# kkty/kmer-sets-compression

Measured on AMD Instinct MI355X. Metric: Mk-mers/s processed in kmerset-multiple-compress; bytes/k-mer after SPSS, higher is better.
Workload: dtype u32

## Files before the change

kmer-sets-compression_amd/csrc/ksh_encode.hip:

```cpp
#include "ksh_internal.h"
#include "ksh_dsu.h"
#include "ksh_kmer.h"

#include <algorithm>
#include <cstddef>
#include <cstdlib>
#include <string>

namespace ksh {

#ifndef KSH_RULER_SHIFT
#define KSH_RULER_SHIFT 5
#endif
constexpr int kRulerShift = KSH_RULER_SHIFT;
constexpr uint32_t kRulerEvery = 1u << kRulerShift;

constexpr uint32_t kNone = 0xFFFFFFFFu;
constexpr uint32_t kMulti = 0xFFFFFFFEu;

#ifndef KSH_JUMP_HOPS
#define KSH_JUMP_HOPS 4
#endif
constexpr int kJumpHops = KSH_JUMP_HOPS;

#ifdef KSH_TRACE
__device__ unsigned long long* g_probe_trace = nullptr;
__device__ long long g_probe_trace_rows = 0;
#define KSH_PMARK(which, m)                                                                              \
  do {                                                                                                   \
    if (g_probe_trace && threadIdx.x == 0 && int64_t(blockIdx.x) < g_probe_trace_rows)                    \
      g_probe_trace[((which) * g_probe_trace_rows + blockIdx.x) * 16 + (m)] = __builtin_amdgcn_s_memtime(); \
  } while (0)
#define KSH_PMARK_WAVE(which)                                                                            \
  do {                                                                                                   \
    if (g_probe_trace && threadIdx.x % 64 == 0 && threadIdx.x / 64 < 16 && int64_t(blockIdx.x) < g_probe_trace_rows) \
      g_probe_trace[((which) * g_probe_trace_rows + blockIdx.x) * 16 + threadIdx.x / 64] = __builtin_amdgcn_s_memtime(); \
  } while (0)
#else
#define KSH_PMARK(which, m) do { } while (0)
#define KSH_PMARK_WAVE(which) do { } while (0)
#endif

template <typename KeyT>
__global__ __launch_bounds__(256) void k_fine_index(const int64_t* __restrict__ off,
                                                     const KeyT* __restrict__ keys, int key_bits,
                                                     int fine_bits, uint32_t* __restrict__ fine,
                                                     int64_t n_buckets) {
  extern __shared__ uint32_t s_fine[];
  const int64_t b = blockIdx.x;
  const int64_t lo = off[b], hi = off[b + 1];
  const int kSlices = 1 << fine_bits;
  const int sh = key_bits - fine_bits;
  uint32_t* f = fine + (b << fine_bits);
  if (lo == hi) {
    for (int sub = threadIdx.x; sub < kSlices; sub += 256) f[sub] = uint32_t(lo);
  } else {
    constexpr int kAhead = 4;
    for (int64_t base = lo; base < hi; base += 256 * kAhead) {
      KeyT cur_key[kAhead], prev_key[kAhead];
#pragma unroll
      for (int u = 0; u < kAhead; u++) {
        const int64_t i = base + u * 256 + threadIdx.x;
        if (i < hi) {
          cur_key[u] = keys[i];
          prev_key[u] = i > lo ? keys[i - 1] : KeyT(0);
        }
      }
#pragma unroll
      for (int u = 0; u < kAhead; u++) {
        const int64_t i = base + u * 256 + threadIdx.x;
        if (i < hi) {
          const int cur = int(uint64_t(cur_key[u]) >> sh);
          const int prev = i > lo ? int(uint64_t(prev_key[u]) >> sh) : -1;
          for (int sub = prev + 1; sub <= cur; sub++) s_fine[sub] = uint32_t(i);
        }
      }
    }
    const int last = int(uint64_t(keys[hi - 1]) >> sh);
    for (int sub = last + 1 + int(threadIdx.x); sub < kSlices; sub += 256) s_fine[sub] = uint32_t(hi);
    __syncthreads();
    for (int sub = threadIdx.x; sub < kSlices; sub += 256) f[sub] = s_fine[sub];
  }
  if (b == n_buckets - 1 && threadIdx.x == 0) fine[n_buckets << fine_bits] = uint32_t(hi);
}

template <typename KeyT>
__global__ __launch_bounds__(256) void k_coarse_index(DevSet<KeyT> set, int64_t n_entries, uint32_t* __restrict__ coarse) {
  const int64_t e = int64_t(blockIdx.x) * blockDim.x + threadIdx.x;
  if (e >= n_entries) return;
  const int64_t t = e << kCoarseShift;
  coarse[e] = uint32_t(set.bucket_search(t < set.n ? t : set.n - 1));
}

template <typename KeyT, bool kDirected, typename F>
__device__ __forceinline__ void for_side_neighbours(const DevSet<KeyT>& set, uint64_t x, uint64_t rx,
                                                    int64_t t, int side, F f) {
  const int k = set.k;
  if (kDirected) {
    if (side) {
      set.for_group4(kmer_next(x, k, 0), [&](int64_t idx) {
        if (idx != t) f(idx, 0u);
      });
    } else {
#pragma unroll
      for (int c = 0; c < 4; c++) {
        const uint64_t z = kmer_prev(x, k, c);
        if (z == x) continue;
        const int64_t idx = set.find(z);
        if (idx >= 0) f(idx, 0u);
      }
    }
    return;
  }
  set.for_group4(kmer_next(side ? x : rx, k, 0), [&](int64_t idx) {
    if (idx != t) f(idx, side ? 0u : 1u);
  });
  const uint64_t base = side ? rx : x;
#pragma unroll
  for (int c = 0; c < 4; c++) {
    const uint64_t z = kmer_prev(base, k, c);
    if (revcomp(z, k) < z) continue;
    if (z == x) continue;
    const int64_t idx = set.find(z);
    if (idx >= 0) f(idx, side ? 1u : 0u);
  }
}

template <typename KeyT, bool kDirected>
__global__ __launch_bounds__(256) void k_adjacency(DevSet<KeyT> set, uint32_t* __restrict__ nbr,
                                                    int* __restrict__ self_rc) {
  __shared__ int64_t s_bucket[2];
  const int64_t t = int64_t(blockIdx.x) * blockDim.x + threadIdx.x;
  const uint64_t x = set.kmer_in_block(t, s_bucket);
  if (t >= set.n) return;
  const uint64_t rx = kDirected ? 0 : revcomp(x, set.k);
  if (!kDirected && rx == x) *self_rc = 1;
  int cnt[2] = {0, 0};
  uint32_t single[2] = {kNone, kNone};
#pragma unroll
  for (int side = 0; side < 2; side++)
    for_side_neighbours<KeyT, kDirected>(set, x, rx, t, side, [&](int64_t idx, uint32_t same) {
      cnt[side]++;
      single[side] = (uint32_t(idx) << 1) | same;
    });
  nbr[2 * t] = cnt[0] == 0 ? kNone : (cnt[0] == 1 ? single[0] : kMulti);
  nbr[2 * t + 1] = cnt[1] == 0 ? kNone : (cnt[1] == 1 ? single[1] : kMulti);
}

template <typename KeyT, bool kDirected>
__global__ __launch_bounds__(256) void k_link_cut(DevSet<KeyT> set, uint32_t* __restrict__ nbr) {
  const int64_t t = int64_t(blockIdx.x) * blockDim.x + threadIdx.x;
  if (t >= set.n) return;
  const uint2 mine = reinterpret_cast<const uint2*>(nbr)[t];
  if (mine.x != kMulti && mine.y != kMulti) return;
  const uint64_t x = set.kmer(t);
  const uint64_t rx = kDirected ? 0 : revcomp(x, set.k);
  for (int side = 0; side < 2; side++) {
    if ((side ? mine.y : mine.x) != kMulti) continue;
    for_side_neighbours<KeyT, kDirected>(set, x, rx, t, side, [&](int64_t idx, uint32_t same) {
      uint32_t* facing = nbr + 2 * idx + (same ? side : side ^ 1);
      if (*reinterpret_cast<volatile uint32_t*>(facing) < kMulti) *reinterpret_cast<volatile uint32_t*>(facing) = kNone;
    });
    nbr[2 * t + side] = kNone;
  }
}

template <typename KeyT>
struct __attribute__((aligned(8))) RcRecord {
  KeyT key;
  uint32_t t;
};

template <typename KeyT>
__global__ __launch_bounds__(1024) void k_rc_hist(const KeyT* __restrict__ keys, int64_t n, int k, int key_bits,
                                                   int nbits, int64_t per_row,
                                                   uint32_t* __restrict__ hist_matrix) {
  extern __shared__ uint32_t lds_hist[];
  const int nb = 1 << nbits;
  for (int b = threadIdx.x; b < nb; b += blockDim.x) lds_hist[b] = 0u;
  __syncthreads();
  const int64_t t_begin = int64_t(blockIdx.x) * per_row;
  const int64_t t_end = min(t_begin + per_row, n);
  const int low_bits = 2 * k - 2 - nbits;
  for (int64_t t = t_begin + threadIdx.x; t < t_end; t += blockDim.x) {
    const uint64_t rx = revcomp(uint64_t(keys[t]), k);
    atomicAdd(&lds_hist[uint32_t(rx >> low_bits) & uint32_t(nb - 1)], 1u);
  }
  __syncthreads();
  uint32_t* my_row = hist_matrix + int64_t(blockIdx.x) * nb;
  for (int b = threadIdx.x; b < nb; b += blockDim.x) my_row[b] = lds_hist[b];
}

constexpr int kColTeams = 16;
__global__ __launch_bounds__(64 * kColTeams) void k_rc_columns(uint32_t* __restrict__ hist_matrix, int64_t n_rows,
                                                                int nb, int64_t* __restrict__ totals) {
  __shared__ uint32_t team_total[kColTeams][64];
  const int lane = threadIdx.x & 63, team = threadIdx.x >> 6;
  const int b = blockIdx.x * 64 + lane;
  const int64_t per_team = (n_rows + kColTeams - 1) / kColTeams;
  const int64_t g0 = min(int64_t(team) * per_team, n_rows), g1 = min(g0 + per_team, n_rows);
  uint32_t run = 0;
  if (b < nb)
    for (int64_t g = g0; g < g1; g++) run += hist_matrix[g * nb + b];
  team_total[team][lane] = run;
  __syncthreads();
  if (b >= nb) return;
  uint32_t before = 0, all = 0;
#pragma unroll
  for (int t2 = 0; t2 < kColTeams; t2++) {
    const uint32_t v = team_total[t2][lane];
    if (t2 < team) before += v;
    all += v;
  }
  run = before;
  for (int64_t g = g0; g < g1; g++) {
    uint32_t* cell = hist_matrix + g * nb + b;
    const uint32_t c = *cell;
    *cell = run;
    run += c;
  }
  if (team == 0) totals[b] = all;
}

template <typename KeyT>
__global__ __launch_bounds__(1024) void k_rc_scatter(DevSet<KeyT> set, int nbits, int round_bits, int round,
                                                      int64_t per_row,
                                                      const uint32_t* __restrict__ hist_matrix,
                                                      const int64_t* __restrict__ goff,
                                                      RcRecord<KeyT>* __restrict__ rec) {
  extern __shared__ uint32_t lds_hist[];
  const int nb = 1 << nbits;
  const uint32_t* my_row = hist_matrix + int64_t(blockIdx.x) * nb;
  for (int b = threadIdx.x; b < nb; b += blockDim.x) lds_hist[b] = uint32_t(goff[b]) + my_row[b];
  const int64_t t_begin = int64_t(blockIdx.x) * per_row;
  const int64_t t_end = min(t_begin + per_row, set.n);
  __syncthreads();
  if (t_begin >= t_end) return;
  const int64_t b_first = set.bucket_of(t_begin), b_last = set.bucket_of(t_end - 1);
  const int k = set.k, low_bits = 2 * set.k - 2 - nbits;
  const uint64_t low_mask = (uint64_t(1) << low_bits) - 1;
  for (int64_t t = t_begin + threadIdx.x; t < t_end; t += blockDim.x) {
    const uint64_t key = uint64_t(set.keys[t]);
    const uint32_t grp = uint32_t(revcomp(key, k) >> low_bits) & uint32_t(nb - 1);
    if (int(grp >> (nbits - round_bits)) != round) continue;
    int64_t lo = b_first, hi = b_last;
    while (lo < hi) {
// ... 1811 lines not shown

__global__ __launch_bounds__(256) void k_end_counts(const uint32_t* __restrict__ link, int64_t n,
                                                     int64_t* __restrict__ counts, uint8_t* __restrict__ flags8) {
  __shared__ uint64_t lds4[4];
  const int64_t t0 = (int64_t(blockIdx.x) * 256 + threadIdx.x) * kHeadItems;
  const uint32_t flags = end_flags8(link, t0, n);
  flags8[int64_t(blockIdx.x) * 256 + threadIdx.x] = uint8_t(flags);
  uint64_t total;
  (void)block_scan_packed(uint64_t(__popc(flags)), lds4, &total);
  if (threadIdx.x == 0) counts[blockIdx.x] = int64_t(total);
}

__global__ __launch_bounds__(256) void k_end_fill(const uint8_t* __restrict__ flags8, int64_t n,
                                                   const int64_t* __restrict__ before,
                                                   uint32_t* __restrict__ ends, uint8_t* __restrict__ hcls) {
  __shared__ uint64_t lds4[4];
  const int64_t t0 = (int64_t(blockIdx.x) * 256 + threadIdx.x) * kHeadItems;
  static_assert(kHeadItems == 8, "one 8-byte store per thread");
  if (t0 + kHeadItems <= n) {
    *reinterpret_cast<uint64_t*>(hcls + t0) = ~uint64_t(0);
  } else {
    for (int64_t t = t0; t < n; t++) hcls[t] = 0xFF;
  }
  const uint32_t flags = flags8[int64_t(blockIdx.x) * 256 + threadIdx.x];
  const uint64_t mine = uint64_t(__popc(flags));
  uint64_t total;
  int64_t at = before[blockIdx.x] + int64_t(block_scan_packed(mine, lds4, &total) - mine);
#pragma unroll
  for (int i = 0; i < kHeadItems; i++)
    if (flags & (1u << i)) ends[at++] = uint32_t(t0 + i);
}

__global__ __launch_bounds__(256) void k_head_block_counts(const uint8_t* __restrict__ hcls, int64_t n,
                                                            int64_t* __restrict__ b01,
                                                            int64_t* __restrict__ b23) {
  __shared__ uint64_t lds4[4];
  const int64_t t0 = (int64_t(blockIdx.x) * 256 + threadIdx.x) * kHeadItems;
  uint8_t c[kHeadItems];
  uint64_t total;
  (void)block_scan_packed(head_counts8(hcls, t0, n, c), lds4, &total);
  if (threadIdx.x == 0) {
    b01[blockIdx.x] = int64_t(total & 0xFFFF) | (int64_t((total >> 16) & 0xFFFF) << 32);
    b23[blockIdx.x] = int64_t((total >> 32) & 0xFFFF) | (int64_t(total >> 48) << 32);
  }
}

__global__ __launch_bounds__(256) void k_unitig_fill(
    const uint8_t* __restrict__ hcls, const int64_t* __restrict__ b01,
    const int64_t* __restrict__ b23, int64_t n, int64_t base1, int64_t base2, int64_t base3,
    const uint8_t* __restrict__ ori, const uint32_t* __restrict__ hlen,
    const uint32_t* __restrict__ hlast, uint32_t* __restrict__ uid, uint32_t* __restrict__ u_head,
    uint32_t* __restrict__ u_first, uint32_t* __restrict__ u_last, uint32_t* __restrict__ u_len) {
  __shared__ uint64_t lds4[4];
  const int64_t t0 = (int64_t(blockIdx.x) * 256 + threadIdx.x) * kHeadItems;
  uint8_t c[kHeadItems];
  const uint64_t mine = head_counts8(hcls, t0, n, c);
  uint64_t total;
  const uint64_t excl = block_scan_packed(mine, lds4, &total) - mine;
  if (mine == 0) return;
  const int64_t w01 = b01[blockIdx.x], w23 = b23[blockIdx.x];
  int64_t next[4] = {(w01 & 0xFFFFFFFF) + int64_t(excl & 0xFFFF),
                     base1 + (w01 >> 32) + int64_t((excl >> 16) & 0xFFFF),
                     base2 + (w23 & 0xFFFFFFFF) + int64_t((excl >> 32) & 0xFFFF),
                     base3 + (w23 >> 32) + int64_t(excl >> 48)};
#pragma unroll
  for (int i = 0; i < kHeadItems; i++) {
    if (c[i] > 3) continue;
    const int64_t t = t0 + i;
    const int64_t u = c[i] == 0 ? next[0]++ : c[i] == 1 ? next[1]++ : c[i] == 2 ? next[2]++ : next[3]++;
    uid[t] = uint32_t(u);
    u_head[u] = uint32_t(t);
    u_first[u] = uint32_t(2 * t) | (ori[t] & 1u);
    u_last[u] = hlast[t];
    u_len[u] = hlen[t];
  }
}

template <typename KeyT>
__global__ __launch_bounds__(256) void k_edges(DevSet<KeyT> set, int64_t n_vertices, bool directed,
                                                const uint32_t* __restrict__ u_first,
                                                const uint32_t* __restrict__ u_last,
                                                const uint32_t* __restrict__ head,
                                                const uint32_t* __restrict__ uid,
                                                uint32_t* __restrict__ edges, uint32_t* __restrict__ mate) {
  const int64_t v = int64_t(blockIdx.x) * blockDim.x + threadIdx.x;
  if (v >= n_vertices) return;
  mate[v] = kNone;
  const uint32_t u = uint32_t(v >> 1), side = uint32_t(v & 1);
  const uint32_t st = side ? u_last[u] : u_first[u];
  const int k = set.k;
  const uint64_t x = set.kmer(st >> 1);
  const uint64_t o = (st & 1) ? revcomp(x, k) : x;
  uint32_t out[4] = {kNone, kNone, kNone, kNone};
  const auto take = [&](int c, int64_t i, bool as_is) {
    const uint32_t u2 = uid[head[i]];
    if (u2 == u) return;
    if (directed) {
      out[c] = 2 * u2 + (side ? 0u : 1u);
      return;
    }
    const uint32_t f = side ? (as_is ? 0u : 1u) : (as_is ? 1u : 0u);
    const uint32_t fs = u_first[u2];
    const uint32_t side2 = ((fs >> 1) == uint32_t(i) && (fs & 1) == f) ? 0u : 1u;
    out[c] = 2 * u2 + side2;
  };
  if (side) {
    set.for_group4(kmer_next(o, k, 0), [&](int64_t i) { take(set.last_base(i), i, true); });
    if (!directed) {
#pragma unroll
      for (int c = 0; c < 4; c++) {
        const uint64_t y = kmer_next(o, k, c), r = revcomp(y, k);
        if (r < y) {
          const int64_t i = set.find(r);
          if (i >= 0) take(c, i, false);
        }
      }
    }
  } else {
#pragma unroll
    for (int c = 0; c < 4; c++) {
      const uint64_t y = kmer_prev(o, k, c);
      if (directed || y <= revcomp(y, k)) {
        const int64_t i = set.find(y);
        if (i >= 0) take(c, i, true);
      }
    }
    if (!directed) {
      const uint64_t ro = revcomp(o, k);
      set.for_group4(kmer_next(ro, k, 0), [&](int64_t i) {
        const int c = 3 - set.last_base(i);
        const uint64_t y = kmer_prev(o, k, c);
        if (revcomp(y, k) < y) take(c, i, false);
      });
    }
  }
  *reinterpret_cast<uint4*>(edges + 4 * v) = make_uint4(out[0], out[1], out[2], out[3]);
}

__device__ __forceinline__ uint64_t slot_priority(uint32_t v, int c, bool directed) {
  if (directed && !(v & 1)) return ~uint64_t(0);
  return uint64_t(v >> 1) * 8 + ((v & 1) ? 0 : 4) + uint64_t(c);
}

__global__ __launch_bounds__(256) void k_match_best(const uint32_t* __restrict__ edges,
                                                     const uint32_t* __restrict__ mate,
                                                     int64_t n_vertices, bool directed,
                                                     unsigned long long* __restrict__ best_prio,
                                                     uint32_t* __restrict__ best_w,
                                                     const int* __restrict__ prev,
                                                     int* __restrict__ any_live) {
  if (prev && *prev == 0) return;
  const int64_t v = int64_t(blockIdx.x) * blockDim.x + threadIdx.x;
  if (v >= n_vertices) return;
  uint32_t bw = kNone;
  uint64_t bp = ~uint64_t(0);
  if (mate[v] == kNone) {
#pragma unroll
    for (int c = 0; c < 4; c++) {
      const uint32_t w = edges[4 * v + c];
      if (w == kNone || mate[w] != kNone) continue;
      uint64_t pr = slot_priority(uint32_t(v), c, directed);
#pragma unroll
      for (int c2 = 0; c2 < 4; c2++) {
        if (edges[4 * int64_t(w) + c2] == uint32_t(v)) {
          const uint64_t p2 = slot_priority(w, c2, directed);
          pr = p2 < pr ? p2 : pr;
        }
      }
      if (pr < bp) {
        bp = pr;
        bw = w;
      }
// ... 646 lines not shown
constexpr int kWalkRoundsMax = 40;
struct EncCtl {
  int64_t tot[3 + kLenSums];
  int self_rc;
  int rc_marks;
  int64_t t2[2];
  int64_t n_bases;
  unsigned long long sc_used;
  unsigned int long_count[2];
  int rc_batched;
  int tgt_extra;
  int jump_live[kJumpRoundsMax + 1];
  int match_live[kMatchBatch + 1];
  int walk_live[kWalkRoundsMax + 1];
};

struct EncPlan {
  int64_t n = 0, n_u = 0, n_strings = 0, n_bases = 0;
  int mode = 0;
  ksh_geom g{};
  ksh_set_view set{};
  uint32_t *nbr = nullptr, *link = nullptr, *head = nullptr, *pos = nullptr, *hlen = nullptr,
           *hlast = nullptr, *uid = nullptr;
  unsigned long long* info = nullptr;
  uint8_t *ori = nullptr, *hcls = nullptr;
  int64_t *c01 = nullptr, *c23 = nullptr;
  uint32_t* fine = nullptr;
  int fine_bits = 0;
  uint32_t* coarse = nullptr;
  size_t nbr_bytes = 0, link_bytes = 0, info_bytes = 0, ori_bytes = 0;
  char* ublock = nullptr;
  uint32_t *u_head = nullptr, *u_first = nullptr, *u_last = nullptr, *u_len = nullptr,
           *edges = nullptr, *mate = nullptr, *best_w = nullptr, *u_sid = nullptr,
           *u_koff = nullptr, *lens = nullptr, *sc_nodes = nullptr, *sc_parent = nullptr,
           *sc_rank = nullptr;
  unsigned long long *best_prio = nullptr, *sc_used = nullptr;
  uint8_t *visited = nullptr, *scls = nullptr, *u_flip = nullptr;
  int64_t *s_nk = nullptr, *sc01 = nullptr, *sc2 = nullptr, *str_start = nullptr;
  EncCtl* ctl = nullptr;
  int rounds = 0;
  int64_t routes = 0;
  bool stamped = true;
  bool directed = false;
  const unsigned long long *rinfo = nullptr, *chain_info = nullptr;
  const uint32_t* ends = nullptr;
  int64_t n_ends = 0;
  WalkLog log_rulers{}, log_heads{};
  bool cover = false;
  ksh_spss_view in{};
  int64_t* in_start = nullptr;
  bool ready = false;
  bool written = false;
  bool ambiguous = false;
};

#define KSH_BOUND(cond)                                                                              \
  do {                                                                                               \
    if (!(cond)) return ::ksh::fail(KSH_INTERNAL, "encode: bound violated: %s (%s:%d)", #cond, __FILE__, __LINE__); \
  } while (0)
static_assert(sizeof(RcRecord<uint16_t>) == 8 && sizeof(RcRecord<uint32_t>) == 8 && sizeof(RcRecord<uint64_t>) == 16,
              "record sizes the scratch layout assumes");

constexpr int64_t kRcRowsMax = 512;
constexpr int64_t kRcWindowBytes = 78 << 10;

inline bool staged_adjacency() {
  static const bool on = [] {
    const char* e = getenv("KSH_ADJACENCY");
    return !(e && std::string(e) == "probe");
  }();
  return on;
}
inline bool rank_with_stamps() {
  static const bool on = [] {
    const char* e = getenv("KSH_RANK");
    return e && std::string(e) == "stamp";
  }();
  return on;
}
inline bool emit_by_walking() {
  static const bool on = [] {
    const char* e = getenv("KSH_EMIT");
    return e && std::string(e) == "walk";
  }();
  return on;
}
inline int64_t l2_threshold() {
  static const int64_t v = [] {
    const char* e = getenv("KSH_L2_MIN");
    return e ? std::max<int64_t>(4096, atoll(e)) : int64_t(1) << 20;
  }();
  return v;
}
inline unsigned nblk(int64_t n) { return unsigned(std::max<int64_t>(1, (n + 255) / 256)); }

void free_plan(ksh_ctx* ctx) {
  EncPlan* p = static_cast<EncPlan*>(ctx->enc_state);
  if (!p) return;
  if (p->ublock) pool_free(ctx, p->ublock);
  delete p;
  ctx->enc_state = nullptr;
}

static bool replaces_unwritten(const ksh_ctx* ctx, bool cover) {
  const EncPlan* o = static_cast<const EncPlan*>(ctx->enc_state);
  return o && o->ready && !o->written && o->cover == cover;
}

void retire_plan(ksh_ctx* ctx) {
  if (EncPlan* p = static_cast<EncPlan*>(ctx->enc_state)) p->ready = false;
}

static int enc_fine_bits(const ksh_geom* g, int64_t n) {
  const int64_t nb = n_buckets(g);
  int fine_bits = 0;
  while (fine_bits < 13 && fine_bits + 2 < key_bits(g) && (int64_t(3) << fine_bits) < 2 * (n / nb + 1)) fine_bits++;
  return fine_bits;
}
static void enc_slot_layout(Carver& c, EncPlan* p, const ksh_geom* g, int64_t n) {
  const int64_t nb = n_buckets(g);
  const int fine_bits = enc_fine_bits(g, n);
  p->nbr = c.take<uint32_t>(size_t(2 * n), &p->nbr_bytes);
  p->link = c.take<uint32_t>(size_t(2 * n), &p->link_bytes);
  p->info = c.take<unsigned long long>(size_t(2 * n), &p->info_bytes);
  p->head = c.take<uint32_t>(size_t(n));
  p->pos = c.take<uint32_t>(size_t(n));
  p->hlen = c.take<uint32_t>(size_t(n));
  p->hlast = c.take<uint32_t>(size_t(n));
  p->uid = c.take<uint32_t>(size_t(n));
  p->ori = c.take<uint8_t>(size_t(n), &p->ori_bytes);
  p->hcls = c.take<uint8_t>(size_t(n));
  p->c01 = c.take<int64_t>(size_t(2 * n));
  p->c23 = p->c01 ? p->c01 + n : nullptr;
  c.pad(2 * round256(size_t(n) * 8) - round256(size_t(2 * n) * 8));
  p->fine = fine_bits >= 2 ? c.take<uint32_t>((size_t(nb) << fine_bits) + 1) : nullptr;
  p->coarse = c.take_if<uint32_t>(n >= 4 * nb, size_t((n >> kCoarseShift) + 2));
  p->ctl = reinterpret_cast<EncCtl*>(c.take<char>(sizeof(EncCtl) + size_t(2 * nb) * 4));
  c.pad(4096);
}
static size_t enc_slot_bytes(const ksh_geom* g, int64_t n) {
  EncPlan measured;
  return layout_bytes([&](Carver& c) { enc_slot_layout(c, &measured, g, n); });
}
static size_t enc_arena_bytes(const ksh_geom* g, int64_t n) {
  const size_t nb = size_t(n_buckets(g));
  size_t bytes = 2 * scan_scratch_bytes(n) - (1u << 16);
  bytes += size_t(n / kHeadSpan + 64) * 8;
  if (nb <= (size_t(1) << 14)) {
    bytes += size_t(kRcRowsMax) * 2 * nb * 4;
    bytes += (2 * nb + 1) * 16;
    bytes += 2 * nb * 280;
    bytes += 8192;
  }
  return bytes;
}
static void unitig_stage_layout(Carver& c, EncPlan* p, size_t n_u) {
  p->u_len = c.take<uint32_t>(n_u);
  p->u_sid = c.take<uint32_t>(n_u);
  p->u_koff = c.take<uint32_t>(n_u);
  p->lens = c.take<uint32_t>(n_u);
  p->sc_nodes = c.take<uint32_t>(n_u);
  p->sc_parent = c.take<uint32_t>(n_u);
  p->sc_rank = c.take<uint32_t>(n_u);
  p->edges = c.take<uint32_t>(8 * n_u);
  p->mate = c.take<uint32_t>(2 * n_u);
  p->best_w = c.take<uint32_t>(2 * n_u);
// ... 224 lines not shown
      p->routes |= per_group > 4096 ? KSH_ROUTE_RC_1024 : per_group > 1024 ? KSH_ROUTE_RC_512
                   : per_group > 256 ? KSH_ROUTE_RC_256 : KSH_ROUTE_RC_64;
      static const int rc1_mode = [] {
        const char* e = getenv("KSH_RC1");
        return !e ? 1 : (std::string(e) == "marks" ? 2 : (std::string(e) == "batched" ? 0 : 1));
      }();
      const bool rc1_marks = rc1_mode == 2;
      const int rc1_cap = rc1_marks ? 0 : int(std::min<int64_t>(Rc1Cfg<KeyT>::kCap, (per_group * 4 / 3 + 263) & ~int64_t(7)));
      const int pass1_cap = rc1_marks ? -1 : rc1_cap;
      const bool with_rc = rc1_mode != 0;
      int rc1_sbits = 6;
      while ((1 << rc1_sbits) < kRc1SlicesMax && (2 << rc1_sbits) <= rc1_cap + 1) rc1_sbits++;
      const size_t rc1_lds = (size_t(4) << rc1_sbits) + size_t(rc1_cap) * Rc1Cfg<KeyT>::kEntryBytes;
      KSH_BOUND(rc1_lds <= size_t(kRc1LdsBytes) && rc1_cap % 8 == 0 && rc1_cap < (2 << rc1_sbits) - 1);
      if (!rc1_marks) p->routes |= KSH_ROUTE_RC1_STREAMED;
      const int rc1_batched = rc1_mode == 0 ? 1 : 0;
#define KSH_LAUNCH_RC(T)                                                                                              \
  do {                                                                                                                \
    if (with_rc)                                                                                                      \
      hipLaunchKernelGGL((k_adj_rc<KeyT, T>), dim3(unsigned(ng)), dim3(T), rc_lds, st, set, gbits, goff, rec, pb, pb0, \
                         cap, rc0, rc1, &ctl->rc_batched, pass1_cap, &ctl->rc_marks);                                 \
    if (!rc1_marks)                                                                                                   \
      hipLaunchKernelGGL((k_adj_rc1<KeyT, T>), dim3(unsigned(ng)), dim3(T), rc1_lds, st, set, gbits, goff, rec, pb,   \
                         pb0, rc1_cap, rc1_sbits, rc1_batched, rc0, rc1, &ctl->rc_batched);                           \
  } while (0)
      if (per_group > 4096)
        KSH_LAUNCH_RC(1024);
      else if (per_group > 1024)
        KSH_LAUNCH_RC(512);
      else if (per_group > 256)
        KSH_LAUNCH_RC(256);
      else
        KSH_LAUNCH_RC(64);
#undef KSH_LAUNCH_RC
      static const int fwd_mode = [] {
        const char* e = getenv("KSH_FWD");
        return !e ? 0 : (std::string(e) == "probe" ? 1 : (std::string(e) == "staged" ? 2 : 0));
      }();
      if (fwd_mode == 1) {
        hipLaunchKernelGGL((k_adj_fwd<KeyT>), dim3(nblk(n)), dim3(256), 0, st, set, rc0, rc1, p->nbr, self_rc_flag);
      } else if (fwd_mode == 0) {
        p->routes |= KSH_ROUTE_FWD_TARGETS;
        constexpr int kTgtChunk = TgtCfg<KeyT>::kChunk, kTgtStreamMax = TgtCfg<KeyT>::kStreamMax;
        const int64_t n_chunks = (n + kTgtChunk - 1) / kTgtChunk;
        const int64_t cap = n / kTgtStreamMax + 1;
        const size_t cut_bytes = size_t((n_chunks + 1) * kTgtBounds + (n_chunks + cap) * 2 * kTgtBounds) * 8 + size_t(cap) * sizeof(TgtTask);
        int64_t* cuts = cut_bytes <= p->info_bytes ? reinterpret_cast<int64_t*>(p->info)
                                                    : static_cast<int64_t*>(arena_alloc(ctx, cut_bytes));
        if (!cuts) return fail(KSH_INTERNAL, "scratch arena too small");
        int64_t* rec = cuts + (n_chunks + 1) * kTgtBounds;
        TgtTask* task = reinterpret_cast<TgtTask*>(rec + (n_chunks + cap) * 2 * kTgtBounds);
        KSH_BOUND(n_chunks >= 1 && n_chunks * kTgtChunk >= n && n < (int64_t(1) << 31));
        hipLaunchKernelGGL((k_tgt_bounds<KeyT>), dim3(nblk((n_chunks + 1) * 8)), dim3(256), 0, st, set, n_chunks, cuts);
        hipLaunchKernelGGL(k_tgt_split, dim3(nblk(n_chunks)), dim3(256), 0, st, cuts, n_chunks, cap, kTgtStreamMax, rec, task,
                           &ctl->tgt_extra);
        hipLaunchKernelGGL((k_tgt_subcuts<KeyT>), dim3(nblk(cap * 8)), dim3(256), 0, st, set, cuts, n_chunks, cap, task,
                           &ctl->tgt_extra, rec);
        hipLaunchKernelGGL((k_adj_fwd_targets<KeyT>), dim3(unsigned(n_chunks + cap)), dim3(kTgtThreads), 0, st, set, rec,
                           n_chunks, &ctl->tgt_extra, rc0, rc1, p->nbr, self_rc_flag);
      } else {
        p->routes |= KSH_ROUTE_FWD_STAGED;
        const int64_t n_chunks = (n + kFwdChunk - 1) / kFwdChunk;
        int64_t* bounds = reinterpret_cast<int64_t*>(p->info);
        KSH_BOUND(size_t(n_chunks + 1) * kFwdBounds * 8 <= p->info_bytes);
        hipLaunchKernelGGL((k_fwd_bounds<KeyT>), dim3(nblk((n_chunks + 1) * 10)), dim3(256), 0, st, set, n_chunks, bounds);
        hipLaunchKernelGGL((k_adj_fwd_staged<KeyT>), dim3(unsigned(n_chunks)), dim3(kFwdChunk), 0, st, set, bounds,
                           rc0, rc1, p->nbr, self_rc_flag);
#ifdef KSH_FWD_DEBUG
        {
          unsigned long long h[8];
          (void)hipStreamSynchronize(st);
          (void)hipMemcpyFromSymbol(h, HIP_SYMBOL(g_fwd_dbg), sizeof(h));
          fprintf(stderr, "fwd dbg: kmers %llu next!usable %llu next-bucket-miss %llu prev!usable %llu prev-bucket-miss %llu "
                          "next-range>cap %llu two-top-bases %llu\n", h[0], h[1], h[2], h[3], h[4], h[5], h[6]);
          unsigned long long z[8] = {};
          (void)hipMemcpyToSymbol(HIP_SYMBOL(g_fwd_dbg), z, sizeof(z));
        }
#endif
      }
    } else {
      hipLaunchKernelGGL((k_adjacency<KeyT, false>), dim3(nblk(n)), dim3(256), 0, st, set, p->nbr, self_rc_flag);
    }
  }
  if (directed)
    hipLaunchKernelGGL((k_link_cut<KeyT, true>), dim3(nblk(n)), dim3(256), 0, st, set, p->nbr);
  else
    hipLaunchKernelGGL((k_link_cut<KeyT, false>), dim3(nblk(n)), dim3(256), 0, st, set, p->nbr);
  const uint32_t* link = p->nbr;
  const int64_t n_hblocks = (n + kHeadSpan - 1) / kHeadSpan;
  int64_t* b01 = p->c23;
  int64_t* b23 = p->c23 + n_hblocks;
  int64_t* d_tot = ctl->tot;
  int64_t* end_before = static_cast<int64_t*>(arena_alloc(ctx, size_t(n_hblocks + 1) * 8));
  if (!end_before) return fail(KSH_INTERNAL, "scratch arena too small");
  uint32_t* ends = p->pos;
  uint8_t* end_flags = p->ori;
  KSH_BOUND(size_t(n_hblocks) * 256 <= p->ori_bytes);
  hipLaunchKernelGGL(k_end_counts, dim3(unsigned(n_hblocks)), dim3(256), 0, st, link, n, end_before, end_flags);
  KSH_TRY(scan_exclusive_i64(ctx, end_before, end_before, n_hblocks, end_before + n_hblocks));
  hipLaunchKernelGGL(k_end_fill, dim3(unsigned(n_hblocks)), dim3(256), 0, st, end_flags, n, end_before, ends, p->hcls);
  p->directed = directed;
  p->ends = ends;
  KSH_HIP(hipMemcpyAsync(ctx->h_pinned, end_before + n_hblocks, 8, hipMemcpyDeviceToHost, st));
  KSH_HIP(hipStreamSynchronize(st));
  const int64_t n_ends = ctx->h_pinned[0];
  p->n_ends = n_ends;
  for (bool stamped = rank_with_stamps(), first_pass = true;; stamped = true, first_pass = false) {
    const int64_t ns2 = 2 * n;
    const int64_t n_dense = 2 * ((n + kRulerEvery - 1) / kRulerEvery);
    unsigned long long* rinfo = stamped ? reinterpret_cast<unsigned long long*>(p->c01) : p->info;
    unsigned long long* chain_info = stamped ? reinterpret_cast<unsigned long long*>(p->c23) : p->info + n_dense;
    {
      Timer timer(ctx, 4, n);
      if (stamped) {
        KSH_HIP(hipMemsetAsync(p->info, 0xFF, size_t(2 * n) * 8, st));
        hipLaunchKernelGGL(k_ruler_walk, dim3(nblk(n_dense)), dim3(256), 0, st, link, ns2, n_dense, rinfo, p->info);
        hipLaunchKernelGGL(k_ruler_heads, dim3(nblk(n_ends)), dim3(256), 0, st, link, ends, n_ends, p->info, chain_info);
      } else {
        WalkLog lr{}, lh{};
        lr.k = lh.k = g->k;
        const size_t used = (size_t(n_dense) + size_t(n)) * 8;
        const size_t log_bytes = size_t(n_dense) * (8 + 4 * kLogMidRulers + 4) + size_t(n_ends) * (8 + 4 * kLogMidHeads + 4) + 64;
        if (!emit_by_walking() && used + log_bytes <= size_t(2 * n) * 8) {
          unsigned long long* at8 = p->info + n_dense + n;
          lr.hdr = at8;
          lh.hdr = at8 + n_dense;
          uint32_t* at4 = reinterpret_cast<uint32_t*>(at8 + n_dense + n_ends);
          lr.mid = at4;
          lh.mid = at4 + size_t(kLogMidRulers) * n_dense;
          lr.long_walkers = lh.long_walkers = lh.mid + size_t(kLogMidHeads) * n_ends;
          lr.long_count = lh.long_count = ctl->long_count;
          lr.long_tag = 0;
          lh.long_tag = kLongHead;
          lr.n_walkers = n_dense;
          lh.n_walkers = n_ends;
          lr.n_mid = kLogMidRulers;
          lh.n_mid = kLogMidHeads;
          KSH_HIP(hipMemsetAsync(at8, 0xFF, size_t(n_dense + n_ends) * 8, st));
          p->routes |= KSH_ROUTE_EMIT_LOGS;
        }
        p->log_rulers = lr;
        p->log_heads = lh;
        KSH_HIP(hipMemsetAsync(rinfo, 0xFF, size_t(n_dense) * 8, st));
        hipLaunchKernelGGL(k_rank_unset, dim3(nblk(n_ends)), dim3(256), 0, st, ends, n_ends, chain_info);
        static const int64_t race_min = [] {
          const char* e = getenv("KSH_RANK_PHASES");
          if (e && std::string(e) == "1") return int64_t(0);
          if (e && std::string(e) == "2") return int64_t(1) << 60;
          const char* m = getenv("KSH_RANK_RACE_MIN");
          return m ? int64_t(atoll(m)) : int64_t(1) << 18;
        }();
        p->routes |= (n_dense >= race_min ? KSH_ROUTE_RANK_ONE_LAUNCH : 0) | (n_ends >= race_min ? KSH_ROUTE_HEADS_ONE_LAUNCH : 0);
        if (n_dense < race_min)
          hipLaunchKernelGGL(k_rank_walk<1>, dim3(nblk(n_dense)), dim3(256), 0, st, link, ns2, n_dense, rinfo, chain_info, lr,
                             static_cast<unsigned long long*>(nullptr), static_cast<unsigned long long*>(nullptr));
        if (n_ends < race_min)
          hipLaunchKernelGGL(k_rank_heads<1>, dim3(nblk(n_ends)), dim3(256), 0, st, link, ends, n_ends, rinfo, chain_info, lh);
        const bool l2_after = n_dense >= l2_threshold();
        hipLaunchKernelGGL(k_rank_walk<2>, dim3(nblk(n_dense)), dim3(256), 0, st, link, ns2, n_dense, rinfo, chain_info, lr,
                           l2_after ? reinterpret_cast<unsigned long long*>(p->hlen) : nullptr,
                           l2_after ? reinterpret_cast<unsigned long long*>(p->hlast) : nullptr);
        hipLaunchKernelGGL(k_rank_heads<2>, dim3(nblk(n_ends)), dim3(256), 0, st, link, ends, n_ends, rinfo, chain_info, lh);
      }
    }
    const bool two_levels = !stamped && n_dense >= l2_threshold();
    const int64_t n_jump = two_levels ? (((n_dense - 1) >> (kL2Shift + 1)) << 1) + 2 : n_dense;
    unsigned long long* r2 = reinterpret_cast<unsigned long long*>(p->uid);
    unsigned long long* l2_head = reinterpret_cast<unsigned long long*>(p->hlen);
    unsigned long long* l2_stamp = reinterpret_cast<unsigned long long*>(p->hlast);
    if (two_levels) p->routes |= KSH_ROUTE_JUMP_TWO_LEVEL;
    if (stamped) p->routes = (p->routes | KSH_ROUTE_RANK_STAMPED) & ~int64_t(KSH_ROUTE_EMIT_LOGS | KSH_ROUTE_RANK_ONE_LAUNCH | KSH_ROUTE_HEADS_ONE_LAUNCH | KSH_ROUTE_JUMP_TWO_LEVEL);
    if (two_levels) {
      hipLaunchKernelGGL(k_l2_walk<true>, dim3(nblk(n_jump)), dim3(256), 0, st, rinfo, n_dense, r2, l2_head, l2_stamp);
      hipLaunchKernelGGL(k_l2_walk<false>, dim3(nblk(n_dense)), dim3(256), 0, st, rinfo, n_dense, r2, l2_head, l2_stamp);
    }
    int max_rounds = 3;
    for (int64_t x = n_jump; x > 1; x /= (kJumpHops + 1)) max_rounds++;
    max_rounds = std::min(max_rounds, kJumpRoundsMax);
    if (!first_pass) {
      KSH_HIP(hipMemsetAsync(ctl->jump_live, 0, sizeof(ctl->jump_live), st));
      KSH_HIP(hipMemsetAsync(d_tot, 0, (3 + kLenSums) * 8, st));
      KSH_HIP(hipMemsetAsync(ctl->long_count, 0, sizeof(ctl->long_count), st));
    }
    for (int round = 0; round < max_rounds; round++) {
      const int* prev = round ? &ctl->jump_live[round - 1] : nullptr;
      if (two_levels)
        hipLaunchKernelGGL(k_l2_jump, dim3(nblk(n_jump)), dim3(256), 0, st, n_jump, r2, prev, &ctl->jump_live[round]);
      else
        hipLaunchKernelGGL(k_ruler_jump, dim3(nblk(n_dense)), dim3(256), 0, st, n_dense, rinfo, prev,
                           &ctl->jump_live[round]);
    }
    if (two_levels)
      hipLaunchKernelGGL(k_l2_resolve, dim3(nblk(n_dense)), dim3(256), 0, st, n_dense, r2, l2_head, l2_stamp, rinfo);
    int* loop_flag = reinterpret_cast<int*>(d_tot + 2 + kLenSums);
    if (stamped) {
      hipLaunchKernelGGL(k_choose, dim3(nblk(n)), dim3(256), 0, st, p->info, rinfo, chain_info, n, directed,
                         p->head, p->pos, p->ori, p->hcls, p->hlen, p->hlast);
      hipLaunchKernelGGL(k_loops, dim3(nblk(n)), dim3(256), 0, st, link, n, p->head, p->pos, p->ori,
                         p->hcls, p->hlen, p->hlast);
    } else {
      hipLaunchKernelGGL(k_choose_ends, dim3(nblk(n_ends)), dim3(256), 0, st, link, ends, n_ends, rinfo, chain_info,
                         directed, p->head, p->ori, p->hcls, p->hlen, p->hlast,
                         reinterpret_cast<unsigned long long*>(d_tot + 2), loop_flag);
      hipLaunchKernelGGL(k_rulers_done, dim3(nblk(n_dense)), dim3(256), 0, st, rinfo, n_dense, loop_flag);
    }
    hipLaunchKernelGGL(k_head_block_counts, dim3(unsigned(n_hblocks)), dim3(256), 0, st, p->hcls, n, b01, b23);
    KSH_TRY(scan_exclusive_i64(ctx, b01, b01, n_hblocks, d_tot));
    KSH_TRY(scan_exclusive_i64(ctx, b23, b23, n_hblocks, d_tot + 1));
    KSH_HIP(hipGetLastError());
    static_assert(offsetof(EncCtl, self_rc) == (3 + kLenSums) * 8 && (4 + kLenSums) <= 64, "one copy: tot + self_rc");
    KSH_HIP(hipMemcpyAsync(ctx->h_pinned, d_tot, (4 + kLenSums) * 8, hipMemcpyDeviceToHost, st));
    KSH_HIP(hipStreamSynchronize(st));
    if (*reinterpret_cast<int*>(ctx->h_pinned + 3 + kLenSums))
      return fail(KSH_INVALID_ARGUMENT, "the canonical set holds a k-mer that is its own reverse "
                                        "complement (even k): not supported");
    static_assert(offsetof(EncCtl, rc_marks) == offsetof(EncCtl, self_rc) + 4, "the word behind self_rc, in the same copy");
    if (reinterpret_cast<int*>(ctx->h_pinned + 3 + kLenSums)[1]) p->routes |= KSH_ROUTE_RC_MARKS_GROUPS;
    p->stamped = stamped;
    p->rinfo = rinfo;
    p->chain_info = chain_info;
    if (stamped) break;
    int64_t accounted = 0;
    for (int i = 0; i < kLenSums; i++) accounted += ctx->h_pinned[2 + i];
    if (accounted == n && *reinterpret_cast<int*>(ctx->h_pinned + 2 + kLenSums) == 0) break;
  }
  const int64_t n0 = ctx->h_pinned[0] & 0xFFFFFFFF, n1 = ctx->h_pinned[0] >> 32;
  const int64_t n2 = ctx->h_pinned[1] & 0xFFFFFFFF, n3 = ctx->h_pinned[1] >> 32;
  const int64_t n_u = n0 + n1 + n2 + n3;
  p->n_u = n_u;

  const auto unitig_block = [&](Carver& c) { enc_unitig_layout(c, p, size_t(n_u)); };
  const size_t ub = layout_bytes(unitig_block);
  KSH_TRY(pool_alloc(ctx, ub, reinterpret_cast<void**>(&p->ublock)));
  KSH_BOUND(layout_bind(p->ublock, ub, unitig_block));
  p->sc_used = &ctl->sc_used;

  hipLaunchKernelGGL(k_unitig_fill, dim3(unsigned(n_hblocks)), dim3(256), 0, st, p->hcls, b01, b23, n, n0,
                     n0 + n1, n0 + n1 + n2, p->ori, p->hlen, p->hlast, p->uid, p->u_head, p->u_first,
                     p->u_last, p->u_len);

  int64_t ns = n_u;
  int walk_rounds = 0;
  if (mode == 1) {
    hipLaunchKernelGGL(k_unitig_strings, dim3(nblk(n_u)), dim3(256), 0, st, p->u_len, n_u, g->k,
                       p->u_sid, p->u_koff, p->u_flip, p->lens, p->str_start);
  } else {
    hipLaunchKernelGGL((k_edges<KeyT>), dim3(nblk(2 * n_u)), dim3(256), 0, st, set, 2 * n_u, directed,
                       p->u_first, p->u_last, p->head, p->uid, p->edges, p->mate);
    KSH_TRY(cover_stage(ctx, p, n_u, directed, mode == 2, g->k, &walk_rounds));
  }
  arena_reset(ctx);
  KSH_TRY(scan_exclusive_i64(ctx, p->str_start, p->str_start, n_u, &ctl->n_bases));
  hipLaunchKernelGGL(k_unitig_place, dim3(nblk(n_u)), dim3(256), 0, st, p->u_len, p->u_sid, p->u_koff,
                     p->u_flip, p->str_start, p->lens, p->u_head, n_u, reinterpret_cast<UnitigPlace*>(p->c01),
                     walk_rounds > 0 ? &ctl->walk_live[walk_rounds - 1] : nullptr);
  KSH_HIP(hipGetLastError());
  constexpr size_t kTail = sizeof(EncCtl) - offsetof(EncCtl, t2);
  static_assert(kTail <= 64 * sizeof(int64_t) && offsetof(EncCtl, n_bases) == offsetof(EncCtl, t2) + 16, "pinned read-back");
  KSH_HIP(hipMemcpyAsync(ctx->h_pinned, ctl->t2, kTail, hipMemcpyDeviceToHost, st));
  KSH_HIP(hipStreamSynchronize(st));
  const int* walk_live_host = reinterpret_cast<const int*>(reinterpret_cast<const char*>(ctx->h_pinned) +
                                                           (offsetof(EncCtl, walk_live) - offsetof(EncCtl, t2)));
  if (walk_rounds > 0 && walk_live_host[walk_rounds - 1])
    return fail(KSH_INTERNAL, "the path cover still holds a loop");
  {
    const char* tail = reinterpret_cast<const char*>(ctx->h_pinned);
    const auto at_tail = [&](size_t member_off) { return tail + (member_off - offsetof(EncCtl, t2)); };
    if (*reinterpret_cast<const int*>(at_tail(offsetof(EncCtl, rc_batched)))) p->routes |= KSH_ROUTE_RC_BATCHED;
    if (*reinterpret_cast<const int*>(at_tail(offsetof(EncCtl, tgt_extra))) > 0) p->routes |= KSH_ROUTE_TGT_PARTS;
    const unsigned int* lc = reinterpret_cast<const unsigned int*>(at_tail(offsetof(EncCtl, long_count)));
    if (!p->stamped && (lc[0] || lc[1])) p->routes |= KSH_ROUTE_LONG_STRETCHES;
    if (p->rounds > kMatchFirst) p->routes |= KSH_ROUTE_MATCH_MORE_ROUNDS;
  }
  if (mode != 1) ns = (ctx->h_pinned[0] & 0xFFFFFFFF) + (ctx->h_pinned[0] >> 32) + ctx->h_pinned[1];
  p->n_strings = ns;
  p->n_bases = ctx->h_pinned[2];
  p->ready = true;
  *n_strings = p->n_strings;
  *n_bases = p->n_bases;
  return KSH_OK;
}

template <typename KeyT>
int encode_write_t(ksh_ctx* ctx, uint64_t* d_words, uint32_t* d_lens) {
  EncPlan* p = static_cast<EncPlan*>(ctx->enc_state);
  if (p->n == 0) return KSH_OK;
  const ksh_geom* g = &p->g;
  const int64_t n = p->n;
  DevSet<KeyT> set{p->set.d_offsets, static_cast<const KeyT*>(p->set.d_keys), n_buckets(g), n, g->k,
                   key_bits(g)};
  set.fine = p->fine;
  set.fine_bits = p->fine_bits;
  set.coarse = p->coarse;
  hipStream_t st = ctx->stream;
  const size_t need = size_t(p->n_bases) + 64;
  uint8_t* bytes;
  void* tmp = nullptr;
  if (need <= size_t(2 * n) * 4) {
    bytes = reinterpret_cast<uint8_t*>(p->link);
  } else {
    KSH_TRY(pool_alloc(ctx, need, &tmp));
    bytes = static_cast<uint8_t*>(tmp);
  }
  {
    Timer timer(ctx, 5, n);
    const UnitigPlace* place = reinterpret_cast<const UnitigPlace*>(p->c01);
    const int64_t n_sampled = (n + kRulerEvery - 1) / kRulerEvery;
#define KSH_EMIT(W, R)                                                                                         \
  do {                                                                                                         \
    if (p->stamped) {                                                                                          \
      hipLaunchKernelGGL((k_emit<KeyT, W>), dim3(nblk(n)), dim3(256), 0, st, set, p->head, p->pos, p->ori,     \
                         place, bytes);                                                                        \
    } else if (p->log_rulers.hdr) {                                                                            \
      hipLaunchKernelGGL((k_emit_log_rulers<KeyT, R>), dim3(kLongBlocks + nblk(p->log_rulers.n_walkers)),      \
                         dim3(256), 0, st, set, p->nbr, p->rinfo, p->chain_info, p->log_rulers, p->log_heads,  \
                         p->directed, p->ends, place, bytes);                                                  \
      hipLaunchKernelGGL((k_emit_log_heads<KeyT, R>), dim3(nblk(p->log_heads.n_walkers)), dim3(256), 0, st,    \
                         set, p->nbr, p->rinfo, p->chain_info, p->log_heads, p->directed, p->ends, place,      \
                         bytes);                                                                               \
    } else {                                                                                                   \
      hipLaunchKernelGGL((k_emit_rulers<KeyT, R>), dim3(nblk(n_sampled)), dim3(256), 0, st, set, p->nbr,       \
                         p->rinfo, p->chain_info, p->directed, place, bytes);                                  \
      hipLaunchKernelGGL((k_emit_heads<KeyT, R>), dim3(nblk(p->n_ends)), dim3(256), 0, st, set, p->nbr,        \
                         p->rinfo, p->chain_info, p->directed, p->ends, p->n_ends, place, bytes);              \
    }                                                                                                          \
  } while (0)
    if (g->k >= 16)
      KSH_EMIT(16, 16);
    else if (g->k >= 8)
      KSH_EMIT(4, 8);
    else if (g->k >= 4)
// ... 278 lines not shown
```

Measured before the change: 27690.

## Mark cut link sides and skip neighbour search for true dead ends in k_edges

k_link_cut now records, in a bitmap, every k-mer side whose link it cuts. It also processes four k-mers per thread using vectorized uint4 loads of the neighbour table. k_edges checks each unitig end: if the link is kNone and the side was never cut, the end has no neighbours at all, so it writes empty edges and skips the k-mer lookup and hash searches. The cost is a memset of the bitmap, atomicOr traffic during cutting, and reuse of the p->link buffer as scratch.

After: 28570 (median of 6 runs). 1.03x the previous value.

```diff
diff --git a/kmer-sets-compression_amd/csrc/ksh_encode.hip b/kmer-sets-compression_amd/csrc/ksh_encode.hip
--- a/kmer-sets-compression_amd/csrc/ksh_encode.hip
+++ b/kmer-sets-compression_amd/csrc/ksh_encode.hip
@@ -6,6 +6,10 @@
 #include <cstddef>
 #include <cstdlib>
 #include <string>
+#ifdef KSH_EDGES_DEBUG
+#include <cstdio>
+#include <vector>
+#endif
 
 namespace ksh {
 
@@ -147,21 +151,52 @@
   nbr[2 * t + 1] = cnt[1] == 0 ? kNone : (cnt[1] == 1 ? single[1] : kMulti);
 }
 
+__device__ __forceinline__ void mark_cut(uint32_t* cut_marks, int64_t entry) {
+  if (cut_marks) atomicOr(cut_marks + (entry >> 5), 1u << (entry & 31));
+}
+constexpr int kCutItems = 4;
+constexpr int kCutSpan = 256 * kCutItems;
 template <typename KeyT, bool kDirected>
-__global__ __launch_bounds__(256) void k_link_cut(DevSet<KeyT> set, uint32_t* __restrict__ nbr) {
-  const int64_t t = int64_t(blockIdx.x) * blockDim.x + threadIdx.x;
-  if (t >= set.n) return;
-  const uint2 mine = reinterpret_cast<const uint2*>(nbr)[t];
-  if (mine.x != kMulti && mine.y != kMulti) return;
-  const uint64_t x = set.kmer(t);
-  const uint64_t rx = kDirected ? 0 : revcomp(x, set.k);
-  for (int side = 0; side < 2; side++) {
-    if ((side ? mine.y : mine.x) != kMulti) continue;
-    for_side_neighbours<KeyT, kDirected>(set, x, rx, t, side, [&](int64_t idx, uint32_t same) {
-      uint32_t* facing = nbr + 2 * idx + (same ? side : side ^ 1);
-      if (*reinterpret_cast<volatile uint32_t*>(facing) < kMulti) *reinterpret_cast<volatile uint32_t*>(facing) = kNone;
-    });
-    nbr[2 * t + side] = kNone;
+__global__ __launch_bounds__(256) void k_link_cut(DevSet<KeyT> set, uint32_t* __restrict__ nbr,
+                                                   uint32_t* __restrict__ cut_marks) {
+  static_assert(kCutItems % 2 == 0, "a pair of k-mers per load");
+  const int64_t t0 = int64_t(blockIdx.x) * kCutSpan + 2 * threadIdx.x;
+  uint4 mine[kCutItems / 2];
+  bool any = false;
+#pragma unroll
+  for (int j = 0; j < kCutItems / 2; j++) {
+    const int64_t t = t0 + 512 * j;
+    if (t + 1 < set.n) {
+      mine[j] = *reinterpret_cast<const uint4*>(nbr + 2 * t);
+    } else if (t < set.n) {
+      const uint2 last = *reinterpret_cast<const uint2*>(nbr + 2 * t);
+      mine[j] = make_uint4(last.x, last.y, kNone, kNone);
+    } else {
+      mine[j] = make_uint4(kNone, kNone, kNone, kNone);
+    }
+    any |= mine[j].x == kMulti || mine[j].y == kMulti || mine[j].z == kMulti || mine[j].w == kMulti;
+  }
+  if (!any) return;
+#pragma unroll
+  for (int i = 0; i < kCutItems; i++) {
+    const uint32_t mine_l = (i & 1) ? mine[i / 2].z : mine[i / 2].x, mine_r = (i & 1) ? mine[i / 2].w : mine[i / 2].y;
+    if (mine_l != kMulti && mine_r != kMulti) continue;
+    const int64_t t = t0 + 512 * (i / 2) + (i & 1);
+    const uint64_t x = set.kmer(t);
+    const uint64_t rx = kDirected ? 0 : revcomp(x, set.k);
+    for (int side = 0; side < 2; side++) {
+      if ((side ? mine_r : mine_l) != kMulti) continue;
+      for_side_neighbours<KeyT, kDirected>(set, x, rx, t, side, [&](int64_t idx, uint32_t same) {
+        const int64_t entry = 2 * idx + (same ? side : side ^ 1);
+        uint32_t* facing = nbr + entry;
+        if (*reinterpret_cast<volatile uint32_t*>(facing) < kMulti) {
+          *reinterpret_cast<volatile uint32_t*>(facing) = kNone;
+          mark_cut(cut_marks, entry);
+        }
+      });
+      nbr[2 * t + side] = kNone;
+      mark_cut(cut_marks, 2 * t + side);
+    }
   }
 }
 
@@ -2139,12 +2174,21 @@
                                                 const uint32_t* __restrict__ u_last,
                                                 const uint32_t* __restrict__ head,
                                                 const uint32_t* __restrict__ uid,
+                                                const uint32_t* __restrict__ link,
+                                                const uint32_t* __restrict__ cut_marks,
                                                 uint32_t* __restrict__ edges, uint32_t* __restrict__ mate) {
   const int64_t v = int64_t(blockIdx.x) * blockDim.x + threadIdx.x;
   if (v >= n_vertices) return;
   mate[v] = kNone;
   const uint32_t u = uint32_t(v >> 1), side = uint32_t(v & 1);
   const uint32_t st = side ? u_last[u] : u_first[u];
+  if (cut_marks) {
+    const int64_t entry = 2 * int64_t(st >> 1) + ((st & 1) ^ side);
+    if (link[entry] == kNone && !((cut_marks[entry >> 5] >> (entry & 31)) & 1u)) {
+      *reinterpret_cast<uint4*>(edges + 4 * v) = make_uint4(kNone, kNone, kNone, kNone);
+      return;
+    }
+  }
   const int k = set.k;
   const uint64_t x = set.kmer(st >> 1);
   const uint64_t o = (st & 1) ? revcomp(x, k) : x;
@@ -2957,6 +3001,13 @@
   static const bool on = [] {
     const char* e = getenv("KSH_EMIT");
     return e && std::string(e) == "walk";
+  }();
+  return on;
+}
+inline bool edges_skip_dead_ends() {
+  static const bool on = [] {
+    const char* e = getenv("KSH_EDGES");
+    return !(e && std::string(e) == "search");
   }();
   return on;
 }
@@ -3347,10 +3398,17 @@
       hipLaunchKernelGGL((k_adjacency<KeyT, false>), dim3(nblk(n)), dim3(256), 0, st, set, p->nbr, self_rc_flag);
     }
   }
+  uint32_t* cut_marks = edges_skip_dead_ends() ? p->link : nullptr;
+  if (cut_marks) {
+    const size_t mark_bytes = size_t((2 * n + 31) / 32) * 4;
+    KSH_BOUND(mark_bytes <= p->link_bytes);
+    KSH_HIP(hipMemsetAsync(cut_marks, 0, mark_bytes, st));
+  }
+  const unsigned cut_blocks = unsigned((n + kCutSpan - 1) / kCutSpan);
   if (directed)
-    hipLaunchKernelGGL((k_link_cut<KeyT, true>), dim3(nblk(n)), dim3(256), 0, st, set, p->nbr);
+    hipLaunchKernelGGL((k_link_cut<KeyT, true>), dim3(cut_blocks), dim3(256), 0, st, set, p->nbr, cut_marks);
   else
-    hipLaunchKernelGGL((k_link_cut<KeyT, false>), dim3(nblk(n)), dim3(256), 0, st, set, p->nbr);
+    hipLaunchKernelGGL((k_link_cut<KeyT, false>), dim3(cut_blocks), dim3(256), 0, st, set, p->nbr, cut_marks);
   const uint32_t* link = p->nbr;
   const int64_t n_hblocks = (n + kHeadSpan - 1) / kHeadSpan;
   int64_t* b01 = p->c23;
@@ -3511,7 +3569,29 @@
                        p->u_sid, p->u_koff, p->u_flip, p->lens, p->str_start);
   } else {
     hipLaunchKernelGGL((k_edges<KeyT>), dim3(nblk(2 * n_u)), dim3(256), 0, st, set, 2 * n_u, directed,
-                       p->u_first, p->u_last, p->head, p->uid, p->edges, p->mate);
+                       p->u_first, p->u_last, p->head, p->uid, link, cut_marks, p->edges, p->mate);
+#ifdef KSH_EDGES_DEBUG
+    if (cut_marks) {
+      const size_t n_sides = size_t(2 * n), n_unitigs = size_t(n_u);
+      std::vector<uint32_t> h_link(n_sides), h_marks((n_sides + 31) / 32), h_first(n_unitigs), h_last(n_unitigs);
+      (void)hipStreamSynchronize(st);
+      (void)hipMemcpy(h_link.data(), link, h_link.size() * 4, hipMemcpyDeviceToHost);
+      (void)hipMemcpy(h_marks.data(), cut_marks, h_marks.size() * 4, hipMemcpyDeviceToHost);
+      (void)hipMemcpy(h_first.data(), p->u_first, h_first.size() * 4, hipMemcpyDeviceToHost);
+      (void)hipMemcpy(h_last.data(), p->u_last, h_last.size() * 4, hipMemcpyDeviceToHost);
+      long long marked = 0, dead = 0, cut = 0, live = 0;
+      for (uint32_t w : h_marks) marked += __builtin_popcount(w);
+      for (int64_t v = 0; v < 2 * n_u; v++) {
+        const uint32_t s = (v & 1) ? h_last[size_t(v >> 1)] : h_first[size_t(v >> 1)];
+        const size_t entry = 2 * size_t(s >> 1) + ((s & 1) ^ uint32_t(v & 1));
+        if (h_link[entry] != kNone) live++;
+        else if ((h_marks[entry >> 5] >> (entry & 31)) & 1u) cut++;
+        else dead++;
+      }
+      fprintf(stderr, "edges dbg: kmers %lld unitig-sides %lld dead-ends %lld cut-ends %lld live-ends %lld marked-sides %lld\n",
+              (long long)n, (long long)(2 * n_u), dead, cut, live, marked);
+    }
+#endif
     KSH_TRY(cover_stage(ctx, p, n_u, directed, mode == 2, g->k, &walk_rounds));
   }
   arena_reset(ctx);
```
